# Pi-Star-Lab/RESCO

Hardware: AMD Instinct MI355X
Metric: env-steps/sec (higher is better)
Workload: dtype f32; 1 GPU; ingolstadt21 x 4096 lock-step envs per GPU (BASELINE config 3), fixed demand from the map's rou.xml, on-device seeded random policy, Krauss sigma 0.5 + speedFactor dev 0.1; tls_expiry=1, map=ingolstadt21, envs_per_gpu=4096, pipes=2, ticks_per_env_step=10, block_threads=512, lds_bytes_per_env=40896, parallelism=env-batch split x1, no collective on the data path

## Files before the change

resco_amd/csrc/resco_step.h:

```cpp
#pragma once
#include "resco_tables.h"

struct State {
    char *base;
    size_t nc;
    int32_t *trip_log;
    int32_t *env;
    int32_t *tls;
    long long *stats;
    uint16_t *dep_next;
    uint32_t *mail;
    RS_HD float *pos() const { return (float *)base; }
    RS_HD float *speed() const { return RS_G((float *)(base + 4 * nc)); }
    RS_HD float *accel() const { return RS_G((float *)(base + 8 * nc)); }
    RS_HD float *tloss() const { return RS_G((float *)(base + 12 * nc)); }
    RS_HD float *sf() const { return RS_G((float *)(base + 16 * nc)); }
    RS_HD uint32_t *coop(int par) const { return RS_G((uint32_t *)(base + (par ? 43 : 20) * nc)); }
    RS_HD uint32_t *cooplead(int par) const { return RS_G((uint32_t *)(base + (par ? 47 : 24) * nc)); }
    RS_HD uint16_t *lane() const { return RS_G((uint16_t *)(base + 28 * nc)); }
    RS_HD uint16_t *trip() const { return RS_G((uint16_t *)(base + 30 * nc)); }
    RS_HD uint16_t *cursor() const { return RS_G((uint16_t *)(base + 32 * nc)); }
    RS_HD uint16_t *swait() const { return RS_G((uint16_t *)(base + 34 * nc)); }
    RS_HD uint16_t *rwait() const { return RS_G((uint16_t *)(base + 36 * nc)); }
    RS_HD uint16_t *depart() const { return RS_G((uint16_t *)(base + 38 * nc)); }
// ... 383 lines not shown

#ifndef RS_LAYOUT_ONLY
template <class F> struct KTabFix {
    const KTab &K;
    const KCold &cold;
    RS_MEM explicit KTabFix(const KTab &K_) : K(K_), cold(K_.cold) {}
#define X(n) static constexpr int32_t n = F::n;
    RS_SCN_KTAB(X)
#undef X
#define X(n) static constexpr float n = __builtin_bit_cast(float, (uint32_t)F::n##_bits);
    RS_SCN_KTAB_F(X)
#undef X
    RS_MEM const LaneRec *lanes() const { return K.lanes(); }
    RS_MEM const LinkRec *links() const { return K.links(); }
    RS_MEM const FoeRec *foes() const { return K.foes(); }
    RS_MEM const RStep *rsteps() const { return K.rsteps(); }
    RS_MEM const float *route_cont() const { return K.route_cont(); }
    RS_MEM const uint16_t *next_link() const { return K.next_link(); }
    RS_MEM const uint16_t *notbest() const { return K.notbest(); }
    RS_MEM const RouteRec *routes() const { return K.routes(); }
    RS_MEM const uint16_t *trip_route() const { return K.trip_route(); }
    RS_MEM const uint8_t *trip_vtype() const { return K.trip_vtype(); }
    RS_MEM const char *dem() const { return K.dem(); }
    RS_MEM const uint32_t *dem_env() const { return K.dem_env(); }
};
template <class F> struct LdsScn {
#define X(n, tp) CPtr<tp, F::o_##n> n;
    RS_SCN_LDS(X)
#undef X
    static constexpr uint32_t gstride = F::gstride, lcap = F::lcap;
    static constexpr float cell_inv = __builtin_bit_cast(float, (uint32_t)F::cell_inv_bits);
};

#ifdef RS_EMU_DEBUG
#define RS_CHAIN_GUARD if (++rs_dbg_chain > 50000000L) { printf("endless chain walk\n"); fflush(stdout); abort(); }
#else
#define RS_CHAIN_GUARD
#endif
#ifndef RS_ASSERT
#define RS_ASSERT(c)
#endif
#ifndef RS_SEC
#define RS_SEC_BEGIN
#define RS_SEC(id) {}
#endif
enum RsCount {
    RC_WALK, RC_HOP2, RC_HOP3, RC_HOP4, RC_MAX_HOPS, RC_ROUTE_END, RC_DEAD_END, RC_STOP_RED, RC_RED_TOO_CLOSE, RC_MINOR_FAR,
    RC_FOE_IN, RC_FOE_BLOCKED, RC_FOE_RED, RC_FOE_ARR, RC_FOE_VIA1, RC_FOE_VIA2, RC_NEXT_LEADER, RC_LOOK_DONE,
    RC_STRATEGIC, RC_SG, RC_SG_LEAD, RC_SG_WANT, RC_URGENT, RC_FOLL_T, RC_CHANGE, RC_LEAD_REQ, RC_COOP_REQ, RC_SWAP, RC_COUNT
};
#ifndef RS_COUNT
#define RS_COUNT(id) {}
#endif
template <class LT> RS_DEV int lane_cells(const LT &L, const LaneRec &LR) { return (int)(LR.len * L.cell_inv) + 1; }
template <class LT> RS_DEV int cell_of(const LT &L, float pos, int ncell) { const int c = (int)(pos * L.cell_inv); return c < ncell ? c : ncell - 1; }

struct Grid { uint16_t *c; uint32_t tag; };
RS_DEV unsigned long long grid_tag4(const Grid &g) { return g.tag ? 0x8000800080008000ull : 0ull; }
RS_DEV int cell_head(const Grid &g, int c) {
    const uint32_t v = g.c[c];
    return ((v ^ g.tag) & CELL_TAG) ? (int)NIL : (int)(v & NIL);
}
RS_DEV uint16_t grid_push(const Grid &g, int c, int s, bool mover) {
    uint32_t *w = (uint32_t *)g.c + (c >> 1);
    const int sh = (c & 1) * 16;
    const uint32_t flag = (mover ? CELL_MOVER : 0u) | g.tag;
    uint32_t old = *w, assumed, cell;
    do {
        assumed = old;
        cell = (assumed >> sh) & 0xFFFFu;
        if ((cell ^ g.tag) & CELL_TAG) cell = NIL;
        const uint32_t keep = cell & CELL_MOVER;
        uint32_t cnt = (cell >> CELL_CNT_SHIFT) & CELL_CNT_MAX;
        if (cnt < CELL_CNT_MAX) cnt += 1u;
        old = rs_atomic_cas(w, assumed, (assumed & ~(0xFFFFu << sh)) | (((uint32_t)s | (cnt << CELL_CNT_SHIFT) | keep | flag) << sh));
    } while (old != assumed);
    return (uint16_t)(cell & NIL);
}
RS_DEV unsigned long long quad_load(const Grid &g, int b) { return *(const unsigned long long *)(g.c + b) ^ grid_tag4(g); }
RS_DEV unsigned long long quad_occ(const Grid &g, int b) {
    const unsigned long long w = quad_load(g, b);
    const unsigned long long x = (w & 0x07FF07FF07FF07FFull) ^ 0x07FF07FF07FF07FFull;
    return (x + 0x07FF07FF07FF07FFull) & 0x0800080008000800ull & ~(w >> 4);
}
RS_DEV int cells_count(const Grid &g, int c0, int nc) {
    const int c1 = c0 + nc - 1;
    int n = 0;
    for (int b = c0 & ~3; b <= c1; b += 4) {
        const unsigned long long w = quad_load(g, b);
        unsigned long long m = (w >> CELL_CNT_SHIFT) & 0x0007000700070007ull;
        m &= ~(((w >> 15) & 0x0001000100010001ull) * 7ull);
        const int lo = c0 - b, hi = c1 - b;
        if (lo > 0) m &= ~0ull << (16 * lo);
        if (hi < 3) m &= ~0ull >> (16 * (3 - hi));
        n += (int)((m * 0x0001000100010001ull) >> 48);
    }
    return n;
}
RS_DEV int scan_up(const Grid &g, int c0, int c1) {
    for (int b = c0 & ~3; b <= c1; b += 4) {
        unsigned long long m = quad_occ(g, b);
        const int lo = c0 - b, hi = c1 - b;
        if (lo > 0) m &= ~0ull << (16 * lo);
        if (hi < 3) m &= ~0ull >> (16 * (3 - hi));
        if (m) return b + ((rs_ffsll(m) - 1) >> 4);
    }
// ... 77 lines not shown
    if (f.slot != NIL && f.pos() > win) f.slot = NIL;
    return f;
}
template <class LT> RS_DEV Found leader_found(const LT &L, const Grid &grid, int cell0, int ncell, float pos, int k, int self, float win) {
    const int c = cell_of(L, pos, ncell);
    const unsigned long long mykey = order_key(pos, k);
    Found f{(int)NIL, ~0ull, 0u, 0u};
    const uint32_t cw = grid.c[cell0 + c];
    int s = ((cw ^ grid.tag) & CELL_TAG) ? (int)NIL : (int)(cw & NIL);
    if (s == self && ((cw >> CELL_CNT_SHIFT) & CELL_CNT_MAX) == 1u) s = NIL;
    while (s != NIL) {
        RS_ASSERT(s != self || order_key(L.node[s].pos, L.node[s].trip) == mykey)
        RS_CHAIN_STEP(f, s, (key > mykey) & (key < f.key))
    }
    if (f.slot == NIL && c + 1 < ncell) {
        const int cc = scan_up(grid, cell0 + c + 1, cell0 + cell_of(L, pos + win, ncell));
        if (cc >= 0) f = chain_rearmost(L, cell_head(grid, cc));
    }
    if (f.slot != NIL && f.pos() - pos > win) f.slot = NIL;
    return f;
}
template <class LT> RS_DEV int leader_within(const LT &L, const Grid &grid, int cell0, int ncell, float pos, int k, int self, float win) {
    return leader_found(L, grid, cell0, ncell, pos, k, self, win).slot;
}
template <class LT> RS_DEV int follower_within(const LT &L, const Grid &grid, int cell0, int ncell, float pos, int k, int self, float win) {
    const int c = cell_of(L, pos, ncell);
    const unsigned long long mykey = order_key(pos, k);
    Found f{(int)NIL, 0ull, 0u, 0u};
    for (int s = cell_head(grid, cell0 + c); s != NIL;) {
        RS_ASSERT(s != self || order_key(L.node[s].pos, L.node[s].trip) == mykey)
        RS_CHAIN_STEP(f, s, (key < mykey) & (key > f.key))
    }
    if (f.slot == NIL && c > 0) {
        const float lo = pos - win;
        const int cc = scan_down(grid, cell0 + (lo > 0.0f ? cell_of(L, lo, ncell) : 0), cell0 + c - 1);
        if (cc >= 0) f = chain_frontmost(L, cell_head(grid, cc));
    }
    if (f.slot != NIL && pos - f.pos() > win) f.slot = NIL;
    (void)self;
    return f.slot;
}
template <class LT> RS_DEV int at_or_behind_within(const LT &L, const Grid &grid, int cell0, int ncell, float back, float win) {
    if (back < 0.0f) return NIL;
    const int c = cell_of(L, back, ncell);
    Found f{(int)NIL, 0ull, 0u, 0u};
    for (int s = cell_head(grid, cell0 + c); s != NIL;) RS_CHAIN_STEP(f, s, !(nd_.pos > back) & (key > f.key))
    if (f.slot == NIL && c > 0) {
        const float lo = back - win;
        const int cc = scan_down(grid, cell0 + (lo > 0.0f ? cell_of(L, lo, ncell) : 0), cell0 + c - 1);
        if (cc >= 0) f = chain_frontmost(L, cell_head(grid, cc));
    }
    if (f.slot != NIL && back - f.pos() > win) f.slot = NIL;
    return f.slot;
}

template <class TT, class LT> RS_DEV int tls_state(const TT &T, const LT &L, int tls, int pos) {
    if (tls == 0xFF) return TLS_G;
    return L.tstate[tls * T.tls_maxl + pos];
}
template <class TT> RS_DEV uint16_t cache_link(const TT &T, const LaneRec &LR, int lane, int rq, int trip) {
    if (LR.link_cnt == 0) return NLINK_NONE;
    if (LR.flags & LF_INTERNAL) { const int l = LR.link_start; return (uint16_t)(l | (rs_at(T.links(), l).arr_idx >= 0 ? NLINK_ARR : 0)); }
    return rs_at(T.next_link(), ((uint32_t)rq * (uint32_t)T.kmax + (uint32_t)(lane - (int)LR.edge_lane0)) * 2u + (uint32_t)(trip & 1));
}
template <class TT, class LT> RS_DEV bool foe_blocked(const TT &T, const LT &L, const Grid &grid, const LinkRec &K) {
    for (int i = K.foe_start; i < K.foe_start + K.foe_cnt; ++i) {
        const FoeRec F = rec_load16(T.foes(), i);
        if (F.tls != 0xFF && tls_state(T, L, F.tls, F.tls_pos) == TLS_R) { RS_COUNT(RC_FOE_RED) continue; }
        if (F.arr_idx >= 0 && L.arr[F.arr_idx] < RM_FOE_GAP_Q) { RS_COUNT(RC_FOE_ARR) return true; }
        if (F.via1_cell0 != 0xFFFF && cells_have_mover(grid, F.via1_cell0, F.via1_nc)) { RS_COUNT(RC_FOE_VIA1) return true; }
        if (F.via2_cell0 != 0xFFFF && cells_have_mover(grid, F.via2_cell0, F.via2_nc)) { RS_COUNT(RC_FOE_VIA2) return true; }
    }
    return false;
}
template <class TT, class LT> RS_DEV void tls_refresh(const TT &T, const LT &L, const KParams &P, int s, int ph) {
    const int w = T.tls_maxl >> 2;
    const uint32_t *src = (const uint32_t *)((P.fixed_program ? T.cold.fix8 + T.cold.fix_state_off[s] : T.cold.tls8 + T.cold.tls_state_off[s]) + ph * T.tls_maxl);
    uint32_t *dst = (uint32_t *)((uint8_t *)L.tstate + s * T.tls_maxl);
    uint32_t v[8];
#pragma unroll
    for (int i = 0; i < 8; ++i) v[i] = src[i < w ? i : 0];
#pragma unroll
    for (int i = 0; i < 8; ++i) if (i < w) dst[i] = v[i];
#pragma unroll 1
    for (int i = 8; i < w; ++i) dst[i] = src[i];
}
template <class TT, class LT> RS_DEV void set_phase(const TT &T, const LT &L, const KParams &P, int s, int ph) {
    if (ph < 0 || ph >= T.cold.tls_nphase[s]) return;
    L.phase[s] = ph;
    L.left[s] = P.tls_expiry ? T.cold.tls_dur[T.cold.tls_dur_off[s] + ph] : RM_TLS_HOLD_TICKS;
    tls_refresh(T, L, P, s, ph);
}
template <class TT, class LT> RS_DEV void tls_begin_of_tick(const TT &T, const LT &L, const KParams &P, int s, int tick) {
    if (P.do_fsm && !P.fixed_program && tick == T.yellow_length) set_phase(T, L, P, s, L.nextp[s]);
    int left = L.left[s];
    if (left == 0) {
        const int32_t *dur = P.fixed_program ? T.cold.fix_dur + T.cold.fix_dur_off[s] : T.cold.tls_dur + T.cold.tls_dur_off[s];
        const int Pn = P.fixed_program ? T.cold.fix_nphase[s] : T.cold.tls_nphase[s];
        const int ph = (L.phase[s] + 1) % Pn;
        left = dur[ph];
        L.phase[s] = ph;
        tls_refresh(T, L, P, s, ph);
    }
    L.left[s] = left - 1;
}
struct ContRow { float c[4]; const float *cn; };
// ... 109 lines not shown
    bool r;
    if ((nb >> kk) & 1u) r = true;
    else if ((((uint32_t)t >> 1) + (uint32_t)k) & 3u) r = false;
    else {
        const int tk = kk + ((t & 1) ? -1 : +1);
        if (tk < 0 || tk >= n) r = false;
        else if (!((nb >> tk) & 1u)) r = true;
        else { float rem; r = strategic_dir(cont_row(T, rq), nb, tk, n, x, v, RM_SG_EXTRA_LANES, rem, OCC_NONE, 0, 0, 0.0f) == 0; }
    }
#ifdef RS_EMU_CHECK_MAIL
    RS_ASSERT(r == may_change_lanes_row(cont_row(T, rq), LR, lane, k, x, v, t))
#endif
    return r;
}
template <class TT, class LT> RS_DEV int classify(const TT &T, const LT &L, int s, const float *vt, float v, float x, const LaneRec &LR, int lane, int rq, uint32_t nb, int k, float sf, int t) {
    int fl = 0;
    if (looks_beyond(vt, v, x, LR.len, LR.vmax, sf)) { fl |= FL_H; list_push(L, L.ls_h, SC_NH, s); }
    if (may_change_lanes(T, rq, nb, LR, lane, k, x, v, t)) { fl |= FL_LC; list_push(L, L.ls_lc, SC_NLC, s); }
    return fl;
}

template <bool LONG, class TT, class LT, class GT> RS_DEV void phase_plan(const TT &T, const LT &L, const Grid &grid, const GT &G, size_t eo, const KParams &P, int genv, int t, int s) {
    RS_SEC_BEGIN
    const Aux ax = L.aux[s];
    const int lane = ax.lane;
    if (lane == (int)LANE_NONE) return;
    const Node me = L.node[s];
    const int k = me.trip;
    const float *vt = L.vtp + me.vt * VT_COLS;
    const float a = vt[VT_ACCEL], b = vt[VT_DECEL], tau = vt[VT_TAU], mingap = vt[VT_MINGAP];
    const float v = me.speed, x = me.pos;
    const float sf = sf_of(me.sfq);
    const LaneRec LR0 = rec_load16(T.lanes(), lane);
    LaneRec LR = LR0;
    float vsafe = RM_BIGF;
    float tgap = 0.0f, tvl = 0.0f, tbl = b;
    bool have = false;
    if (LONG) RS_SEC(7)
    const float vfree = plan_vfree(vt, v, LR.vmax, sf);
    const float look = plan_look(vt, vfree);
    const Found ld = leader_found(L, grid, LR.cell0, lane_cells(L, LR), x, k, s, look + T.maxlen);
    const int lead = ld.slot;
    if (LONG) RS_SEC(8)
    bool found = false;
    if (lead != NIL) {
        const float *vo = L.vtp + ld.vt() * VT_COLS;
        tgap = ld.pos() - vo[VT_LENGTH] - x - mingap;
        tvl = ld.speed(); tbl = vo[VT_DECEL];
        have = true; found = true;
    }
    if (me.sfq & SFQ_MAIL((t + 1) & 1)) {
        const int q = (t + 1) & 1;
        const uint32_t c1 = G.coop(q)[eo + s], c2 = G.cooplead(q)[eo + s];
        if (c1 != COOP_NONE) { G.coop(q)[eo + s] = COOP_NONE; follow_neighbour(T, L, c1, false, LR, lane, x, v, b, tau, mingap, vsafe); }
        if (c2 != COOP_NONE) { G.cooplead(q)[eo + s] = COOP_NONE; follow_neighbour(T, L, c2, true, LR, lane, x, v, b, tau, mingap, vsafe); }
        mail_flag_clear(L, s, q);
    }
#ifdef RS_EMU_CHECK_MAIL
    else { RS_ASSERT(G.coop((t + 1) & 1)[eo + s] == COOP_NONE && G.cooplead((t + 1) & 1)[eo + s] == COOP_NONE) }
#endif
    if (LONG) RS_SEC(9)
    float seen = LR.len - x;
    RS_ASSERT(LONG || found || !(seen < look))
    if (LONG && !found && seen < look) {
        int rq = ax.rq;
        int link = (int)(ax.nlink & 0x7FFF);
        int cur_lane = lane;
        const float bgv = d_brake_gap(v, b);
        RS_COUNT(RC_WALK)
        bool go = true;
        for (int hop = 0; go && hop < RM_MAX_HOPS; ++hop) {
            if (hop == 1) RS_COUNT(RC_HOP2)
            if (hop == 2) RS_COUNT(RC_HOP3)
            if (hop >= 3) RS_COUNT(RC_HOP4)
            const bool cur_int = (LR.flags & LF_INTERNAL) != 0;
            if (hop > 0) link = (int)(cache_link(T, LR, cur_lane, rq, k) & 0x7FFF);
            const bool none = link == NLINK_NONE;
            const LinkRec K = link_load(T.links(), none ? 0 : link);
            const bool sig = !none & (K.tls != 0xFF);
            const int st0 = L.tstate[sig ? K.tls * T.tls_maxl + K.tls_pos : 0];
            const int st = sig ? st0 : (int)TLS_G;
            bool route_end = false;
            if (none) route_end = !cur_int && rs_at(T.rsteps(), rq).next_edge == 0xFFFF;
            const bool red = (st == TLS_R) | (st == TLS_Y);
            const bool red_stop = red & (seen >= bgv);
            const bool minor = !none & !red_stop & !(K.flags & KF_CONT) & (((K.flags & KF_MINOR) != 0) | (st == TLS_g));
            const bool far = minor & (seen > RM_VIS_DIST);
            bool stop_here = (none & !route_end) | red_stop | far;
            if (none & route_end) RS_COUNT(RC_ROUTE_END)
            if (none & !route_end) RS_COUNT(RC_DEAD_END)
            if (red_stop) RS_COUNT(RC_STOP_RED)
            if (red & !red_stop) RS_COUNT(RC_RED_TOO_CLOSE)
            if (far) RS_COUNT(RC_MINOR_FAR)
            if (minor && !far && K.foe_cnt > 0) {
                RS_COUNT(RC_FOE_IN)
                if (foe_blocked(T, L, grid, K)) { RS_COUNT(RC_FOE_BLOCKED) stop_here = true; }
            }
            {
                const float g = seen - RM_STOP_OFFSET;
                tgap = stop_here ? (g > 0.0f ? g : 0.0f) : tgap; tvl = stop_here ? 0.0f : tvl; tbl = stop_here ? b : tbl;
            }
            const bool cont = !none & !stop_here;
            bool hit = false;
            if (cont) {
                LR = K.dest;
                cur_lane = K.to_lane;
                {
                    const float vnl = LR.vmax * sf;
                    if (vnl < vfree) {
                        const float vs = d_free_speed(seen, vnl, b);
                        if (vs < vsafe) vsafe = vs;
                    }
                }
                const Found od = rearmost_within(L, grid, LR.cell0, lane_cells(L, LR), look - seen + T.maxlen);
                hit = od.slot != NIL;
                const float *vo = L.vtp + od.vt() * VT_COLS;
                tgap = hit ? seen + od.pos() - vo[VT_LENGTH] - mingap : tgap;
                tvl = hit ? od.speed() : tvl; tbl = hit ? vo[VT_DECEL] : tbl;
                rq += cur_int ? 0 : 1;
                seen += LR.len;
            }
            have |= stop_here | hit;
            if (hit) RS_COUNT(RC_NEXT_LEADER)
            if (cont & !hit & !(seen < look)) RS_COUNT(RC_LOOK_DONE)
            go = cont & !hit & (seen < look);
        }
        if (go) RS_COUNT(RC_MAX_HOPS)
    }
    if (LONG) RS_SEC(10)
    if (have) {
        const float vs = d_follow_speed(tgap, tvl, b, tbl, tau);
        if (vs < vsafe) vsafe = vs;
    }
    float vmin_n = v - b; if (vmin_n < 0.0f) vmin_n = 0.0f;
    float vmin_e = v - vt[VT_EMERGENCY]; if (vmin_e < 0.0f) vmin_e = 0.0f;
    const float lo = vsafe > vmin_e ? vsafe : vmin_e;
    const float vmin = vmin_n < lo ? vmin_n : lo;
    float vmax = vfree < vsafe ? vfree : vsafe;
    if (vmax < vmin) vmax = vmin;
    const float sigma = P.sigma >= 0.0f ? P.sigma : vt[VT_SIGMA];
    float vd = vmax;
    if (sigma > 0.0f) {
        const float r = d_u01(d_hash(P.seed, (uint32_t)genv, (uint32_t)k, (uint32_t)t, 0u));
        if (vd < a) vd -= sigma * vd * r; else vd -= sigma * a * r;
        if (vd < 0.0f) vd = 0.0f;
    }
    const float vnext = vd > vmin ? vd : vmin;
    L.vnx[s] = vnext;
#ifdef RS_EMU_DEBUG
    if (s == rs_dbg_slot && (t == rs_dbg_t || rs_dbg_t < 0))
        printf("plan t %d slot %d lane %d x %.3f v %.3f lead %d have %d tgap %.3f tvl %.3f vsafe %.3f vfree %.3f vnext %.3f nlink %x\n", t, s, lane, x, v, lead,
               (int)have, tgap, tvl, vsafe, vfree, vnext, ax.nlink);
#endif
    if (LONG) RS_SEC(3)
    if (x + vnext > LR0.len) flag_mover(L, s, t);
    if (LONG) RS_SEC(15)
    (void)LR;
}

template <bool LONG, class TT, class LT, class GT> RS_DEV void phase_move(const TT &T, const LT &L, const Grid &gnew, const GT &G, const KParams &P, int env, size_t eo,
                       int t, bool last_tick, bool more, int s, int &active, int &halted, int &top) {
    const Aux ax = L.aux[s];
    const Node me = L.node[s];
    const int k = me.trip;
    int lane = ax.lane;
#ifdef RS_EMU_DEBUG
    {
        static int moved_at[65536];
        if (moved_at[s] == t + 1) { printf("slot %d moved twice in tick %d: fl %x lane %d trip %d\n", s, t, me.fl, lane, k); fflush(stdout); abort(); }
        moved_at[s] = t + 1;
    }
#endif
#ifdef RS_FIELD_LOADS
    LaneRec LR = rec_load16(T.lanes(), lane);
#endif
    uint32_t nb = rs_at(T.notbest(), ax.rq);
    uint32_t kw = 0;
    if (more && (ax.nlink & NLINK_ARR)) kw = link_reg_word(T, ax.nlink);
    const float sfv = sf_of(me.sfq);
    float tl = G.tloss()[eo + s];
#ifndef RS_FIELD_LOADS
    LaneRec LR = rec_load16(T.lanes(), lane);
#endif
    const int sw = ax.swait;
    int swn = sw;
    const float vn = L.vnx[s];
    int rq = ax.rq;
    uint16_t nlink = ax.nlink;
    int link = (int)(nlink & 0x7FFF);
    bool relink = false;
    int side = 0;
    RS_ASSERT(LONG || (!(me.fl & (LCT_LEFT | LCT_RIGHT | LCT_SWAP_LEFT | LCT_SWAP_RIGHT)) && !(me.pos + vn > LR.len)))
    if (LONG && (me.fl & (LCT_LEFT | LCT_RIGHT | LCT_SWAP_LEFT | LCT_SWAP_RIGHT))) {
        if ((me.fl & (LCT_LEFT | LCT_RIGHT)) && !(me.pos + vn > LR.len)) side = (me.fl & LCT_LEFT) ? +1 : -1;
        else if (me.fl & (LCT_SWAP_LEFT | LCT_SWAP_RIGHT)) side = (me.fl & LCT_SWAP_LEFT) ? +1 : -1;
    }
    if (LONG && side) {
        lane += side;
        LR = rec_load16(T.lanes(), lane);
        nlink = cache_link(T, LR, lane, rq, k);
        link = (int)(nlink & 0x7FFF);
        relink = true;
    }
    const float vref = LR.vmax * sfv;
    if (last_tick && (P.out_mask & OUT_VEH_ACCEL)) G.accel()[eo + s] = vn - me.speed;
    if (vn <= RM_HALT_SPEED) {
        if (sw < 65535) swn = sw + 1;
        halted += 1;
        if (G.trip_log) { const int wt = G.wtot()[eo + s]; if (wt < 65535) G.wtot()[eo + s] = (uint16_t)(wt + 1); }
    } else swn = 0;
    if (vref > 0.0f && vn < vref) { tl += RS_DIV(vref - vn, vref); G.tloss()[eo + s] = tl; }
    float x = me.pos + vn;
    bool arrived = false;
    if (LONG) for (int it = 0; it < 16; ++it) {
        if (!(x > LR.len)) break;
        const bool li = (LR.flags & LF_INTERNAL) != 0;
        if (link == NLINK_NONE) {
            if (!li && rs_at(T.rsteps(), rq).next_edge == 0xFFFF) arrived = true; else x = LR.len;
            break;
        }
        x -= LR.len;
        if (!li) rq += 1;
        {
            const LinkRec Km = link_load(T.links(), link);
            lane = Km.to_lane;
            LR = Km.dest;
        }
        nlink = cache_link(T, LR, lane, rq, k);
        link = (int)(nlink & 0x7FFF);
        relink = true;
    }
    if (LONG && arrived) {
        Aux na = ax; na.lane = LANE_NONE; na.swait = 0;
        L.aux[s] = na;
        L.node[s].trip = TRIP_NONE; L.node[s].fl = (uint8_t)(me.fl & fl_mh(t));
        rs_atomic_and(&L.alive[s >> 5], ~(1u << (s & 31)));
        {
            const int ow = G.owner()[eo + s];
            if (ow != (int)OWNER_NONE) rs_atomic_add(&L.sig_dep[ow], 1);
        }
        G.owner()[eo + s] = OWNER_NONE; G.rwait()[eo + s] = 0;
        rs_atomic_add(&L.sc[SC_NACT], -1);
        rs_atomic_add(&L.sc[SC_STATS + ST_ARRIVED], 1);
        rs_atomic_add(&L.sc[SC_STATS + ST_DURATION], t + 1 - (int)G.depart()[eo + s]);
        rs_atomic_add(&L.sc[SC_STATS + ST_TLOSS], (int)(tl * 1024.0f + 0.5f));
        if (G.trip_log) {
            int32_t *r = G.trip_log + ((size_t)env * T.n_trips + k) * 4;
            r[0] = (int)G.depart()[eo + s]; r[1] = t + 1; r[2] = (int)(tl * 1024.0f + 0.5f); r[3] = (int)G.wtot()[eo + s];
        }
        return;
    }
    active += 1;
    if (s + 1 > top) top = s + 1;
    Aux na = ax;
    na.lane = (uint16_t)lane; na.rq = (uint16_t)rq; na.swait = (uint16_t)swn;
    if (LONG && relink) na.nlink = nlink;
    L.aux[s] = na;
    Node nn = me;
    nn.pos = x; nn.speed = vn; nn.fl = (uint8_t)(me.fl & fl_mh(t));
    nn.nxt = grid_push(gnew, LR.cell0 + cell_of(L, x, lane_cells(L, LR)), s, vn > RM_HALT_SPEED);
    if (more) {
        if (LONG && relink) { nb = rs_at(T.notbest(), rq); if (na.nlink & NLINK_ARR) kw = link_reg_word(T, na.nlink); }
        nn.fl |= classify(T, L, s, L.vtp + me.vt * VT_COLS, vn, x, LR, lane, rq, nb, k, sfv, t + 1);
        L.node[s] = nn;
        if ((na.nlink & NLINK_ARR) && vn > RM_HALT_SPEED) register_approach_w(T, L, kw, vn, x, LR.len, me.vt);
    } else L.node[s] = nn;
    (void)P;
}

template <class LT> RS_DEV int overlapping(const LT &L, const Grid &grid, int cell0, int ncell, float pos, int k, int self, float len_self) {
    const int lead = leader_within(L, grid, cell0, ncell, pos, k, self, RM_NB_WINDOW);
    if (lead != NIL && L.node[lead].pos - L.vtp[L.node[lead].vt * VT_COLS + VT_LENGTH] - pos < 0.0f) return lead;
    const int foll = follower_within(L, grid, cell0, ncell, pos, k, self, RM_NB_WINDOW);
    if (foll != NIL && pos - len_self - L.node[foll].pos < 0.0f) return foll;
    return NIL;
}

template <class TT, class LT, class GT> RS_DEV int phase_lc_decide(const TT &T, const LT &L, const Grid &grid, const GT &G, size_t eo, int t, int s, const Aux &ax, const Node &me) {
    const int lane = ax.lane;
#ifdef RS_FIELD_LOADS
    const LaneRec LR = rec_load16(T.lanes(), lane);
    const ContRow R = cont_row(T, ax.rq);
#else
    const ContRow R = cont_row(T, ax.rq);
    const LaneRec LR = rec_load16(T.lanes(), lane);
#endif
    const uint32_t nbm = rs_at(T.notbest(), ax.rq);
    const int my_wait = (int)ax.swait;
    const int n = LR.flags >> 2;
    if ((LR.flags & LF_INTERNAL) || n < 2) return 0;
    const int dir_allowed = (t & 1) ? -1 : +1;
    const int l0 = LR.edge_lane0, kk = lane - l0;
    const int k = me.trip;
    const float *vt = L.vtp + me.vt * VT_COLS;
    const float x = me.pos, v = me.speed;
    const int nc = lane_cells(L, LR);
    int want = 0, dir = dir_allowed;
    float rem;
    const int sdir = strategic_dir(R, nbm, kk, n, x, v, 0, rem, grid, LR.cell0, nc, T.occ_unit);
    if (sdir != 0) { RS_COUNT(RC_STRATEGIC) dir = sdir; want = 2; }
    int code = 0;
    const int tk = kk + dir;
    if (tk >= 0 && tk < n) {
        const int tcell0 = (int)LR.cell0 + dir * nc;
        int lead_t = NIL, foll_t = NIL;
        bool sg = false;
        if (!want && !((((uint32_t)t >> 1) + (uint32_t)k) & 3u)) {
            float rem_t;
            sg = strategic_dir(R, nbm, tk, n, x, v, RM_SG_EXTRA_LANES, rem_t, grid, tcell0, nc, T.occ_unit) == 0;
        }
        int lead_c = NIL;
        if (sg) { RS_COUNT(RC_SG) lead_c = leader_within(L, grid, LR.cell0, nc, x, k, s, RM_NB_WINDOW); }
        const bool sgl = sg && lead_c != NIL;
        if (want || sgl) lead_t = leader_within(L, grid, tcell0, nc, x, k, s, RM_NB_WINDOW);
        if (sgl) {
            RS_COUNT(RC_SG_LEAD)
            const float gcur = L.node[lead_c].pos - L.vtp[L.node[lead_c].vt * VT_COLS + VT_LENGTH] - x;
            float gtgt = RM_BIGF;
            if (lead_t != NIL) gtgt = L.node[lead_t].pos - L.vtp[L.node[lead_t].vt * VT_COLS + VT_LENGTH] - x;
            if (gcur < v * 3.0f + 15.0f && gtgt > gcur + RM_SG_ADVANTAGE) { RS_COUNT(RC_SG_WANT) want = 1; }
        }
        if (want) {
            foll_t = follower_within(L, grid, tcell0, nc, x, k, s, RM_NB_WINDOW);
            const bool urgent = want == 2 && rem <= RM_URGENT_DIST;
            if (urgent) RS_COUNT(RC_URGENT)
            if (foll_t != NIL) RS_COUNT(RC_FOLL_T)
            bool safe = true;
            if (lead_t != NIL) {
                const Node ld = L.node[lead_t];
                const float *vo = L.vtp + ld.vt * VT_COLS;
                const float gap = ld.pos - vo[VT_LENGTH] - x - (urgent ? 0.0f : vt[VT_MINGAP]);
                const float dec = urgent ? vt[VT_EMERGENCY] : vt[VT_DECEL];
                float vb = v - dec; if (vb < 0.0f) vb = 0.0f;
                if (gap < 0.0f || vb > d_follow_speed(gap, ld.speed, vt[VT_DECEL], vo[VT_DECEL], vt[VT_TAU])) safe = false;
            }
            if (safe && foll_t != NIL) {
                const Node fd = L.node[foll_t];
                const float *vo = L.vtp + fd.vt * VT_COLS;
                const float gap = x - vt[VT_LENGTH] - fd.pos - (urgent ? 0.0f : vo[VT_MINGAP]);
                const float dec = urgent ? vo[VT_EMERGENCY] : vo[VT_DECEL];
                float vb = fd.speed - dec; if (vb < 0.0f) vb = 0.0f;
                if (gap < 0.0f || vb > d_follow_speed(gap, v, vo[VT_DECEL], vt[VT_DECEL], vo[VT_TAU])) safe = false;
            }
            if (safe) {
                if (dir == dir_allowed) { RS_COUNT(RC_CHANGE) code = dir > 0 ? LCT_LEFT : LCT_RIGHT; }
            } else if (want == 2) {
                if (lead_t != NIL) { RS_COUNT(RC_LEAD_REQ) G.cooplead(t & 1)[eo + s] = ((uint32_t)L.node[lead_t].trip << 16) | (uint32_t)lead_t; mail_flag_set(L, s, t & 1); }
                const int R = at_or_behind_within(L, grid, tcell0, nc, x - vt[VT_LENGTH], RM_COOP_RANGE);
                if (R != NIL) { RS_COUNT(RC_COOP_REQ) rs_atomic_min(&G.coop(t & 1)[eo + R], ((uint32_t)k << 16) | (uint32_t)s); mail_flag_set(L, R, t & 1); }
            }
        }
    }
    if (sdir != 0 && (t % RM_SWAP_EVERY) == 0 && v <= RM_HALT_SPEED && rem <= RM_URGENT_DIST &&
        my_wait >= RM_SWAP_WAIT) {
        const int b = overlapping(L, grid, (int)LR.cell0 + sdir * nc, nc, x, k, s, vt[VT_LENGTH]);
        if (b != NIL) {
            const Node nb = L.node[b];
            float rem_b;
            if (nb.speed <= RM_HALT_SPEED && (int)L.aux[b].swait >= RM_SWAP_WAIT &&
                strategic_dir(cont_row(T, L.aux[b].rq), rs_at(T.notbest(), L.aux[b].rq), kk + sdir, n, nb.pos, nb.speed, 0, rem_b, grid, (int)LR.cell0 + sdir * nc, nc, T.occ_unit) == -sdir && rem_b <= RM_URGENT_DIST &&
                overlapping(L, grid, LR.cell0, nc, nb.pos, nb.trip, b, L.vtp[nb.vt * VT_COLS + VT_LENGTH]) == s)
                { RS_COUNT(RC_SWAP) code |= sdir > 0 ? LCT_SWAP_LEFT : LCT_SWAP_RIGHT; }
        }
    }
        return code;
}

template <class TT, class DT, class LT> RS_DEV bool phase_insert_decide(const TT &T, const DT &D, const LT &L, const Grid &grid, int t, int d) {
    if ((int)L.dep_t[d] > t) return false;
    const int k = L.dep[d];
    const DepInfo LR = rec_load8(T.cold.dep_info, d);
    const float *vt = L.vtp + rs_at(D.trip_vtype(), k) * VT_COLS;
    const float mypos = vt[VT_LENGTH] < LR.len ? vt[VT_LENGTH] : LR.len;
    const int nc = (int)(LR.len * L.cell_inv) + 1;
    const int c1 = LR.cell0 + cell_of(L, mypos + vt[VT_MINGAP] + T.maxlen, nc);
    for (int c = scan_up(grid, LR.cell0, c1); c >= 0; c = (c < c1 ? scan_up(grid, c + 1, c1) : -1))
        for (int o = cell_head(grid, c); o != NIL;) { RS_CHAIN_GUARD
            const Node od = L.node[o];
            const float back = (od.pos + L.vnx[o]) - L.vtp[od.vt * VT_COLS + VT_LENGTH];
            if (back - mypos - vt[VT_MINGAP] < 0.0f) return false;
            o = od.nxt;
        }
    return true;
}

template <class LT> RS_DEV int nth_free_slot(const LT &L, int C, int r) {
#pragma unroll 1
    for (int w = 0; w < (C + 31) / 32; ++w) {
        uint32_t fr = ~L.alive0[w];
        if (w == (C - 1) / 32 && (C & 31)) fr &= (1u << (C & 31)) - 1u;
        const int c = rs_popc(fr);
        if (r >= c) { r -= c; continue; }
#pragma unroll 1
        for (int j = 0; j < r; ++j) fr &= fr - 1u;
        return w * 32 + rs_ffs(fr) - 1;
    }
    return -1;
}

template <class TT, class LT, class GT> RS_DEV void lc_decide_and_flag(const TT &T, const LT &L, const Grid &grid, const GT &G, size_t eo, int t, int s) {
    const Aux ax = L.aux[s];
    if (ax.lane == LANE_NONE) return;
    const int code = phase_lc_decide(T, L, grid, G, eo, t, s, ax, L.node[s]);
    if (code) flag_mover(L, s, t, code);
}
struct ExecInline {};

template <int CAP, bool DEM, class Exec, class LT, class TT, class GT>
RS_DEV void rs_step_body_on(Exec &ex, const LT &L, const TT &T, const GT &G, const Out &O, const KParams &P,
                            const int32_t *actions, int env) {
#ifdef RS_DEM_RUNTIME
    const Demand<2, TT> D(T, env);
#else
    const Demand<DEM, TT> D(T, env);
#endif
    const int B = ex.B;
    const int C = CAP ? CAP : T.capacity, S = T.n_signals, NO = T.n_obs;
    const int genv = P.env_base + env;
    const size_t eo = (size_t)env * C;
    const int n_ticks = P.n_ticks;

    uint16_t *const grid0 = L.grid;

    ex.phase(0, [&](int tid) {
        if (tid < SC_STATS + ST_N) L.sc[tid] = tid < 4 ? G.env[env * 4 + tid] : 0;
        for (int i = tid; i < T.n_vtypes * VT_COLS; i += B) L.vtp[i] = T.cold.vtype_params[i];
        for (int i = tid; i < (int)(L.gstride >> 1); i += B) ((uint32_t *)grid0)[i] = 0x07FF07FFu;
        for (int i = tid; i < T.n_arr; i += B) L.arr[i] = ARR_NONE;
        for (int i = tid; i < (C + 31) / 32; i += B) { L.alive[i] = 0u; L.mailw[i] = 0u; }
        for (int i = tid; i < (T.n_dep + 31) / 32; i += B) L.insm[i] = 0u;
        for (int i = tid; i < T.n_dep; i += B) {
            const int k = G.dep_next[(size_t)env * T.n_dep + i];
            L.dep[i] = (uint16_t)k;
            L.dep_t[i] = k == (int)TRIP_NONE ? (uint16_t)0xFFFF : (uint16_t)D.trip_depart()[k];
        }
        for (int i = tid; i < S; i += B) {
            const int ph = G.tls[(env * S + i) * TLS_W + 0];
            L.phase[i] = ph;
            L.left[i] = G.tls[(env * S + i) * TLS_W + 1];
            L.nextp[i] = G.tls[(env * S + i) * TLS_W + 2];
            L.sig_arr[i] = 0; L.sig_dep[i] = G.tls[(env * S + i) * TLS_W + 3];
            tls_refresh(T, L, P, i, ph);
        }
    });
    ex.phase(1, [&](int tid) {
        const int hw0 = L.sc[SC_HW];
        for (int s = tid; s < C; s += B) {
            uint16_t ln = LANE_NONE, tr = TRIP_NONE;
            if (s < hw0) { ln = G.lane()[eo + s]; tr = G.trip()[eo + s]; }
            Aux ax; ax.lane = ln; ax.rq = 0; ax.nlink = NLINK_NONE; ax.swait = 0;
            if (ln == LANE_NONE) { L.aux[s] = ax; L.node[s].trip = TRIP_NONE; continue; }
            const float sp = G.speed()[eo + s], x = G.pos()[eo + s];
            const int rq = (int)T.routes()[D.trip_route()[tr]].start + (int)G.cursor()[eo + s];
            const LaneRec LR0 = rec_load16(T.lanes(), ln);
            ax.rq = (uint16_t)rq;
            ax.nlink = cache_link(T, LR0, ln, rq, tr);
            ax.swait = G.swait()[eo + s];
            L.aux[s] = ax;
            Node nn; nn.pos = x; nn.speed = sp; nn.trip = tr; nn.vt = D.trip_vtype()[tr];
            nn.fl = 0; nn.sfq = (uint16_t)speed_factor_q(P, genv, tr, L.vtp + nn.vt * VT_COLS);
            if ((G.mail[(size_t)env * ((C + 31) / 32) + (s >> 5)] >> (s & 31)) & 1u) nn.sfq |= (uint16_t)SFQ_MAIL((L.sc[SC_T] + 1) & 1);
            nn.nxt = grid_push(Grid{grid0, 0u}, LR0.cell0 + cell_of(L, x, lane_cells(L, LR0)), s, sp > RM_HALT_SPEED);
            if (n_ticks > 0) nn.fl = (uint8_t)classify(T, L, s, L.vtp + nn.vt * VT_COLS, sp, x, LR0, ln, rq, rs_at(T.notbest(), rq), tr, sf_of(nn.sfq), L.sc[SC_T]);
            L.node[s] = nn;
            rs_atomic_or(&L.alive[s >> 5], 1u << (s & 31));
        }
        for (int s = B - 1 - tid; s < S; s += B) {
            if (P.do_fsm && !P.fixed_program) {
                const int a = actions[env * S + s], cur = L.phase[s], Gn = T.cold.tls_ngreen[s];
                if (a < 0 || a >= T.cold.tls_nphase[s]) L.nextp[s] = cur;
                else {
                    L.nextp[s] = a;
                    if (cur != a && cur < Gn && a < Gn) {
                        const int y = T.cold.tls_yellow[T.cold.tls_yel_off[s] + cur * Gn + a];
                        if (y >= 0) set_phase(T, L, P, s, y);
                    }
                }
            }
            if (n_ticks > 0) tls_begin_of_tick(T, L, P, s, 0);
        }
    });
    if (n_ticks > 0) ex.phase(2, [&](int tid) {
        const int hw = L.sc[SC_HW];
        for (int s = tid; s < hw; s += B) {
            const Aux ax = L.aux[s];
            if (ax.lane == LANE_NONE) continue;
            const Node me = L.node[s];
            register_approach(T, L, ax.nlink, me.speed, me.pos, T.lanes()[ax.lane].len, me.vt);
        }
    });

    int cur = 0;
    for (int tick = 0; tick < n_ticks; ++tick) {
        const int t = L.sc[SC_T], hw = L.sc[cur ? SC_HWNEW : SC_HW];
        const Grid gold{grid0, cur ? CELL_TAG : 0u}, gnew{grid0, cur ? 0u : CELL_TAG};
        const bool more = tick + 1 < n_ticks;
        const int lcap = (int)L.lcap;
        const int nwv = B >> 6;
        ex.phase(4, [&](int tid) {
            const int wv = ex.wave_of(tid), ln = tid & 63;
            const int nh = L.sc[SC_NH], nlc = L.sc[SC_NLC];
            const unsigned long long r0 = ex.role_begin();
            int role = 0;
            if (nh > lcap || nlc > lcap) {
                for (int pass = 0; pass < 2; ++pass)
                    for (int w = tid; w < hw; w += B) {
                        if (pass && !(L.node[w].fl & FL_LC)) continue;
                        if (pass) lc_decide_and_flag(T, L, gold, G, eo, t, w);
                        else phase_plan<true>(T, L, gold, G, eo, P, genv, t, w);
                    }
            } else {
                const int hch = (nh + RS_H_CHUNK - 1) / RS_H_CHUNK, lch = (nlc + RS_LIST_CHUNK - 1) / RS_LIST_CHUNK;
                const int total = hch + lch + ((hw + 63) >> 6);
                for (int it = 0;; ++it) {
// ... 282 lines not shown
```

Measured before the change: 4.403 million env-steps/s.

## Merge follower and behind-vehicle scans, branchless lane handoff, loop the swap overlap checks

Replaces the two separate rear-neighbour grid walks (follower_within and at_or_behind_within) with a single combined scan that finds both in one pass over the cell chains. The lane-handoff loop in phase_move is rewritten to avoid early-exit branches, selecting fields with ternaries and always issuing the link load. The swap check's two overlapping() calls are folded into a non-unrolled two-pass loop to shrink inlined code. It also adds optional debug counters. The aim is fewer grid traversals and less branch divergence and code size, at the cost of the handoff loop doing an unconditional link load and more select instructions on each iteration.

```diff
diff --git a/resco_amd/csrc/resco_step.h b/resco_amd/csrc/resco_step.h
--- a/resco_amd/csrc/resco_step.h
+++ b/resco_amd/csrc/resco_step.h
@@ -459,6 +459,15 @@
 #ifndef RS_COUNT
 #define RS_COUNT(id) {}
 #endif
+enum RsCount2 {
+    RC2_MAIL_NO_LOOK, RC2_MAIL_LOOK, RC2_MAIL_COOP, RC2_MAIL_LEAD, RC2_MAIL_RESTORED,
+    RC2_REAR_BOTH, RC2_REAR_ONE, RC2_REAR_NEITHER, RC2_REAR_DIFFER, RC2_REAR_CONT_FOLL, RC2_REAR_CONT_BEHIND,
+    RC2_SWAP_IN, RC2_SWAP_OVERLAP, RC2_SWAP_PASS2, RC2_SWAP,
+    RC2_HAND1, RC2_HAND2, RC2_HAND3, RC2_ARRIVED, RC2_DEAD_END_CLAMP, RC2_COUNT
+};
+#ifndef RS_COUNT2
+#define RS_COUNT2(id) {}
+#endif
 template <class LT> RS_DEV int lane_cells(const LT &L, const LaneRec &LR) { return (int)(LR.len * L.cell_inv) + 1; }
 template <class LT> RS_DEV int cell_of(const LT &L, float pos, int ncell) { const int c = (int)(pos * L.cell_inv); return c < ncell ? c : ncell - 1; }
 
@@ -642,6 +651,39 @@
     }
     if (f.slot != NIL && back - f.pos() > win) f.slot = NIL;
     return f.slot;
+}
+struct RearPair { int foll, behind; };
+template <class LT> RS_DEV RearPair rear_pair_within(const LT &L, const Grid &grid, int cell0, int ncell, float pos, int k, float win_f, float back, float win_b) {
+    const int c = cell_of(L, pos, ncell);
+    const float lo_f = pos - win_f, lo_b = back - win_b;
+    const int cf = cell0 + (lo_f > 0.0f ? cell_of(L, lo_f, ncell) : 0), cb = back < 0.0f ? 0x7FFFFFFF : cell0 + (lo_b > 0.0f ? cell_of(L, lo_b, ncell) : 0);
+    unsigned long long fkey = order_key(pos, k);
+    float rback = back;
+    Found f{(int)NIL, 0ull, 0u, 0u}, r{(int)NIL, 0ull, 0u, 0u};
+    int cc = cell0 + c;
+    bool go = true, first = true;
+    while (go) {
+        fkey = cc >= cf ? fkey : 0ull; rback = cc >= cb ? rback : -1.0f;
+        for (int s = cell_head(grid, cc); s != NIL;) {
+            RS_CHAIN_GUARD
+            const Node nd = node_load(L, s);
+            const unsigned long long key = order_key(nd.pos, nd.trip);
+            const bool tf = (key < fkey) & (key > f.key), tr = !(nd.pos > rback) & (key > r.key);
+            f.slot = tf ? s : f.slot; f.key = tf ? key : f.key;
+            r.slot = tr ? s : r.slot; r.key = tr ? key : r.key;
+            s = nd.nxt;
+        }
+        const bool need_f = (f.slot == NIL) & (cc > cf), need_r = (r.slot == NIL) & (cc > cb);
+        const int lo = need_f ? (need_r && cb < cf ? cb : cf) : cb;
+        go = need_f | need_r;
+        if (first & go & need_f) RS_COUNT2(RC2_REAR_CONT_FOLL)
+        if (first & go & need_r) RS_COUNT2(RC2_REAR_CONT_BEHIND)
+        first = false;
+        cc = scan_down(grid, go ? lo : cc, cc - 1); go = cc >= 0;
+    }
+    if (f.slot != NIL && pos - f.pos() > win_f) f.slot = NIL;
+    if (r.slot != NIL && back - r.pos() > win_b) r.slot = NIL;
+    return RearPair{f.slot, r.slot};
 }
 
 template <class TT, class LT> RS_DEV int tls_state(const TT &T, const LT &L, int tls, int pos) {
@@ -857,8 +899,9 @@
     if (me.sfq & SFQ_MAIL((t + 1) & 1)) {
         const int q = (t + 1) & 1;
         const uint32_t c1 = G.coop(q)[eo + s], c2 = G.cooplead(q)[eo + s];
-        if (c1 != COOP_NONE) { G.coop(q)[eo + s] = COOP_NONE; follow_neighbour(T, L, c1, false, LR, lane, x, v, b, tau, mingap, vsafe); }
-        if (c2 != COOP_NONE) { G.cooplead(q)[eo + s] = COOP_NONE; follow_neighbour(T, L, c2, true, LR, lane, x, v, b, tau, mingap, vsafe); }
+        if (LR.len - x < look) RS_COUNT2(RC2_MAIL_LOOK) else RS_COUNT2(RC2_MAIL_NO_LOOK)
+        if (c1 != COOP_NONE) { RS_COUNT2(RC2_MAIL_COOP) G.coop(q)[eo + s] = COOP_NONE; follow_neighbour(T, L, c1, false, LR, lane, x, v, b, tau, mingap, vsafe); }
+        if (c2 != COOP_NONE) { RS_COUNT2(RC2_MAIL_LEAD) G.cooplead(q)[eo + s] = COOP_NONE; follow_neighbour(T, L, c2, true, LR, lane, x, v, b, tau, mingap, vsafe); }
         mail_flag_clear(L, s, q);
     }
 #ifdef RS_EMU_CHECK_MAIL
@@ -963,6 +1006,14 @@
     (void)LR;
 }
 
+RS_DEV LaneRec lane_rec_select(bool c, const LaneRec &a, const LaneRec &b) {
+    LaneRec r;
+    r.len = c ? a.len : b.len; r.vmax = c ? a.vmax : b.vmax;
+    r.link_start = c ? a.link_start : b.link_start; r.link_cnt = c ? a.link_cnt : b.link_cnt; r.flags = c ? a.flags : b.flags;
+    r.cell0 = c ? a.cell0 : b.cell0; r.edge_lane0 = c ? a.edge_lane0 : b.edge_lane0;
+    return r;
+}
+
 template <bool LONG, class TT, class LT, class GT> RS_DEV void phase_move(const TT &T, const LT &L, const Grid &gnew, const GT &G, const KParams &P, int env, size_t eo,
                        int t, bool last_tick, bool more, int s, int &active, int &halted, int &top) {
     const Aux ax = L.aux[s];
@@ -1017,23 +1068,34 @@
     if (vref > 0.0f && vn < vref) { tl += RS_DIV(vref - vn, vref); G.tloss()[eo + s] = tl; }
     float x = me.pos + vn;
     bool arrived = false;
-    if (LONG) for (int it = 0; it < 16; ++it) {
-        if (!(x > LR.len)) break;
-        const bool li = (LR.flags & LF_INTERNAL) != 0;
-        if (link == NLINK_NONE) {
-            if (!li && rs_at(T.rsteps(), rq).next_edge == 0xFFFF) arrived = true; else x = LR.len;
-            break;
-        }
-        x -= LR.len;
-        if (!li) rq += 1;
-        {
-            const LinkRec Km = link_load(T.links(), link);
-            lane = Km.to_lane;
-            LR = Km.dest;
-        }
-        nlink = cache_link(T, LR, lane, rq, k);
-        link = (int)(nlink & 0x7FFF);
-        relink = true;
+    if (LONG) {
+        bool go = x > LR.len;
+        int handed = 0;
+        for (int it = 0; go && it < 16; ++it) {
+            const bool li = (LR.flags & LF_INTERNAL) != 0;
+            const bool none = link == NLINK_NONE;
+            const LinkRec Km = link_load(T.links(), none ? 0 : link);
+            bool route_end = false;
+            if (none) route_end = !li && rs_at(T.rsteps(), rq).next_edge == 0xFFFF;
+            if (none & !route_end) RS_COUNT2(RC2_DEAD_END_CLAMP)
+            arrived = none & route_end;
+            x = none ? (route_end ? x : LR.len) : x - LR.len;
+            rq += (none | li) ? 0 : 1;
+            lane = none ? lane : (int)Km.to_lane;
+            LR = lane_rec_select(none, LR, Km.dest);
+            const uint16_t nl = cache_link(T, LR, lane, rq, k);
+            RS_ASSERT(!none || nl == nlink)
+            nlink = nl;
+            link = (int)(nlink & 0x7FFF);
+            relink |= !none;
+            handed += none ? 0 : 1;
+            go = !none & (x > LR.len);
+        }
+        if (handed == 1) RS_COUNT2(RC2_HAND1)
+        if (handed == 2) RS_COUNT2(RC2_HAND2)
+        if (handed >= 3) RS_COUNT2(RC2_HAND3)
+        if (arrived) RS_COUNT2(RC2_ARRIVED)
+        (void)handed;
     }
     if (LONG && arrived) {
         Aux na = ax; na.lane = LANE_NONE; na.swait = 0;
@@ -1126,7 +1188,18 @@
             if (gcur < v * 3.0f + 15.0f && gtgt > gcur + RM_SG_ADVANTAGE) { RS_COUNT(RC_SG_WANT) want = 1; }
         }
         if (want) {
-            foll_t = follower_within(L, grid, tcell0, nc, x, k, s, RM_NB_WINDOW);
+            const RearPair rp = rear_pair_within(L, grid, tcell0, nc, x, k, RM_NB_WINDOW, want == 2 ? x - vt[VT_LENGTH] : -1.0f, RM_COOP_RANGE);
+            foll_t = rp.foll;
+#ifdef RS_EMU_CHECK_MAIL
+            RS_ASSERT(foll_t == follower_within(L, grid, tcell0, nc, x, k, s, RM_NB_WINDOW))
+            RS_ASSERT(want != 2 || rp.behind == at_or_behind_within(L, grid, tcell0, nc, x - vt[VT_LENGTH], RM_COOP_RANGE))
+#endif
+            if (want == 2) {
+                if (rp.foll != NIL && rp.behind != NIL) RS_COUNT2(RC2_REAR_BOTH)
+                if ((rp.foll != NIL) != (rp.behind != NIL)) RS_COUNT2(RC2_REAR_ONE)
+                if (rp.foll == NIL && rp.behind == NIL) RS_COUNT2(RC2_REAR_NEITHER)
+                if (rp.foll != NIL && rp.behind != NIL && rp.foll != rp.behind) RS_COUNT2(RC2_REAR_DIFFER)
+            }
             const bool urgent = want == 2 && rem <= RM_URGENT_DIST;
             if (urgent) RS_COUNT(RC_URGENT)
             if (foll_t != NIL) RS_COUNT(RC_FOLL_T)
@@ -1151,21 +1224,34 @@
                 if (dir == dir_allowed) { RS_COUNT(RC_CHANGE) code = dir > 0 ? LCT_LEFT : LCT_RIGHT; }
             } else if (want == 2) {
                 if (lead_t != NIL) { RS_COUNT(RC_LEAD_REQ) G.cooplead(t & 1)[eo + s] = ((uint32_t)L.node[lead_t].trip << 16) | (uint32_t)lead_t; mail_flag_set(L, s, t & 1); }
-                const int R = at_or_behind_within(L, grid, tcell0, nc, x - vt[VT_LENGTH], RM_COOP_RANGE);
+                const int R = rp.behind;
                 if (R != NIL) { RS_COUNT(RC_COOP_REQ) rs_atomic_min(&G.coop(t & 1)[eo + R], ((uint32_t)k << 16) | (uint32_t)s); mail_flag_set(L, R, t & 1); }
             }
         }
     }
     if (sdir != 0 && (t % RM_SWAP_EVERY) == 0 && v <= RM_HALT_SPEED && rem <= RM_URGENT_DIST &&
         my_wait >= RM_SWAP_WAIT) {
-        const int b = overlapping(L, grid, (int)LR.cell0 + sdir * nc, nc, x, k, s, vt[VT_LENGTH]);
-        if (b != NIL) {
-            const Node nb = L.node[b];
-            float rem_b;
-            if (nb.speed <= RM_HALT_SPEED && (int)L.aux[b].swait >= RM_SWAP_WAIT &&
-                strategic_dir(cont_row(T, L.aux[b].rq), rs_at(T.notbest(), L.aux[b].rq), kk + sdir, n, nb.pos, nb.speed, 0, rem_b, grid, (int)LR.cell0 + sdir * nc, nc, T.occ_unit) == -sdir && rem_b <= RM_URGENT_DIST &&
-                overlapping(L, grid, LR.cell0, nc, nb.pos, nb.trip, b, L.vtp[nb.vt * VT_COLS + VT_LENGTH]) == s)
-                { RS_COUNT(RC_SWAP) code |= sdir > 0 ? LCT_SWAP_LEFT : LCT_SWAP_RIGHT; }
+        RS_COUNT2(RC2_SWAP_IN)
+        const int scell0 = (int)LR.cell0 + sdir * nc;
+        int cell0 = scell0, who = s, trip = k, b = NIL;
+        float pos = x, len = vt[VT_LENGTH];
+        bool ok = true;
+#pragma unroll 1
+        for (int pass = 0; ok && pass < 2; ++pass) {
+            const int o = overlapping(L, grid, cell0, nc, pos, trip, who, len);
+            if (pass == 0) {
+                b = o;
+                ok = b != NIL;
+                if (ok) {
+                    RS_COUNT2(RC2_SWAP_OVERLAP)
+                    const Node nb = L.node[b];
+                    float rem_b;
+                    ok = nb.speed <= RM_HALT_SPEED && (int)L.aux[b].swait >= RM_SWAP_WAIT &&
+                         strategic_dir(cont_row(T, L.aux[b].rq), rs_at(T.notbest(), L.aux[b].rq), kk + sdir, n, nb.pos, nb.speed, 0, rem_b, grid, scell0, nc, T.occ_unit) == -sdir && rem_b <= RM_URGENT_DIST;
+                    cell0 = LR.cell0; who = b; trip = nb.trip; pos = nb.pos; len = L.vtp[nb.vt * VT_COLS + VT_LENGTH];
+                    if (ok) RS_COUNT2(RC2_SWAP_PASS2)
+                }
+            } else if (o == s) { RS_COUNT(RC_SWAP) RS_COUNT2(RC2_SWAP) code |= sdir > 0 ? LCT_SWAP_LEFT : LCT_SWAP_RIGHT; }
         }
     }
         return code;
@@ -1264,7 +1350,7 @@
             L.aux[s] = ax;
             Node nn; nn.pos = x; nn.speed = sp; nn.trip = tr; nn.vt = D.trip_vtype()[tr];
             nn.fl = 0; nn.sfq = (uint16_t)speed_factor_q(P, genv, tr, L.vtp + nn.vt * VT_COLS);
-            if ((G.mail[(size_t)env * ((C + 31) / 32) + (s >> 5)] >> (s & 31)) & 1u) nn.sfq |= (uint16_t)SFQ_MAIL((L.sc[SC_T] + 1) & 1);
+            if ((G.mail[(size_t)env * ((C + 31) / 32) + (s >> 5)] >> (s & 31)) & 1u) { RS_COUNT2(RC2_MAIL_RESTORED) nn.sfq |= (uint16_t)SFQ_MAIL((L.sc[SC_T] + 1) & 1); }
             nn.nxt = grid_push(Grid{grid0, 0u}, LR0.cell0 + cell_of(L, x, lane_cells(L, LR0)), s, sp > RM_HALT_SPEED);
             if (n_ticks > 0) nn.fl = (uint8_t)classify(T, L, s, L.vtp + nn.vt * VT_COLS, sp, x, LR0, ln, rq, rs_at(T.notbest(), rq), tr, sf_of(nn.sfq), L.sc[SC_T]);
             L.node[s] = nn;
```

Measured after the change: 4.436 million env-steps/s, median of 6. Within noise of the previous version (+0.8%).
